# cboin1996/avddpg

Hardware: AMD Instinct MI355X
Metric: env-steps/sec + DDPG updates/sec, 4096x5-vehicle platoons (higher is better)
Workload: dtype f32-class (fp16 hi+lo operand pairs on the 16-bit matrix cores, f32 accumulate)

## Files before the change

avddpg_amd/csrc/fsplit.hip:

```cpp
#include <type_traits>

#include "fset_common.h"

namespace avd {
namespace fsplit {
using namespace fset;

struct ActorS {
    static constexpr int K = 256, KP = 256, NFT = 8, NKS = 16, LD = 264, NGT = 9, KG = 288;
    static constexpr bool critic = false;
};
struct CriticS {
    static constexpr int K = 304, KP = 320, NFT = 10, NKS = 19, LD = 312, NGT = 10, KG = 320;
    static constexpr bool critic = true;
};
constexpr int NGT_MAX = 10;

template <int I, int N, class F>
__device__ __forceinline__ void static_for(F&& f) {
    if constexpr (I < N) {
        f(std::integral_constant<int, I>{});
        static_for<I + 1, N>(f);
    }
}
// ... 273 lines not shown
            for (int k = 0; k < 4; ++k) w[k] = k < a.S ? W[k * H1 + f] : 0.f;
            b = th[(critic ? L.cbs : L.ab1) + f];
        }
        if (not_finite(w[0]) || not_finite(w[1]) || not_finite(w[2]) || not_finite(w[3]) || not_finite(b)) atomicOr(a.bad, 1);
        if (S1 * fmaxf(fmaxf(fabsf(w[0]), fabsf(w[1])), fmaxf(fmaxf(fabsf(w[2]), fabsf(w[3])), fabsf(b))) >= F16_OVERFLOW) atomicOr(a.bad, 1);
    }
    a.wf1h[net][((long)set * NGT_MAX + ft) * 64 + lane] = make_wh(w[0], w[1], w[2], w[3], b, S1, h);
    if (net == 1 && ft == 0 && lane < 48) {
        const int hl = lane / 24, hh = (lane / 12) & 1, ks = (lane / 4) % 3, m = lane & 3;
        unsigned v = 0;
#pragma unroll
        for (int e = 0; e < 2; ++e) {
            const int jj = 2 * m + e, fa = 16 * ks + 8 * (jj >> 2) + 4 * hh + (jj & 3);
            f16 hi, lo;
            split1h(S1 * th[L.cWa + fa], hi, lo);
            v |= (unsigned)__builtin_bit_cast(unsigned short, hl ? lo : hi) << (16 * e);
        }
        a.wap[(long)set * 48 + lane] = v;
    }
}

enum HeadMode { OUT_TANH = 0, OUT_TD = 1, HEAD_BOTH = 5, OUT_TANH_SAVE = 6 };
struct HeadArgs {
    unsigned long long* stamp;
    NetP net;
    int n_agents, n_sets;
    const f16x8* xf;
    const float* act;
    const float* act2;
    const float* r;
    const float* yin;
    const float* aw;
    float* out;
    f16* sm;
    float* g3;
    float* dmu;
    float* part_s;
    float* part_s2;
    float* part_m;
    float* tz;
    float gamma, high, inv_n;
    int* bad;
    int abl;
};
#ifndef HEAD_FAST
#define HEAD_FAST 5
#define HEAD_SLOW 3
#endif

template <int S, class NET, int MODE>
__global__ __launch_bounds__(NT) void head_kernel(const HeadArgs p) {
    constexpr int K = NET::K, NKS = NET::NKS, NFT = NET::NFT, LD = NET::LD;
    constexpr int NTH = NT;
    constexpr bool BOTH = (MODE == HEAD_BOTH);
    static_assert(!BOTH || NET::critic, "HEAD_BOTH is a critic mode");
    __shared__ __attribute__((aligned(16))) f16 wimg[2][H2 * LD];
    __shared__ __attribute__((aligned(16))) float b2s[H2];
    __shared__ __attribute__((aligned(16))) float c3s[H2];
    __shared__ __attribute__((aligned(16))) unsigned waps[BOTH ? 48 : 4];
    const int tid = threadIdx.x, w = tid >> 6, lane = tid & 63, r = lane & 31, h = lane >> 5, q = w >> 1, rh = w & 1;
    const int set = blockIdx.x % p.n_sets, j0 = blockIdx.x / p.n_sets, J = gridDim.x / p.n_sets, P = p.n_agents / p.n_sets;
    for (int i = tid; i < 2 * H2 * (K / 8); i += NTH) {
        const int hl = i / (H2 * (K / 8)), rem = i - hl * (H2 * (K / 8)), n = rem / (K / 8), c = rem - n * (K / 8);
        const f16* src = (hl ? p.net.Wlo : p.net.Whi) + ((long)set * H2 + n) * K + 8 * c;
        *(uint4*)(&wimg[hl][n * LD + 8 * c]) = *(const uint4*)src;
    }
    const float* vec = p.net.vec + (long)set * VEC;
// ... 63 lines not shown
            if (FSPLIT_ABL(p.abl) & 4) {
#pragma unroll
                for (int m = 0; m < 8; ++m) ph[m] = __float_as_uint(p1[2 * m]), pl[m] = __float_as_uint(p1[2 * m + 1]);
                return;
            }
#pragma unroll
            for (int m = 0; m < 8; ++m) split2h(relu(p1[2 * m]), relu(p1[2 * m + 1]), ph[m], pl[m]);
        };
        auto zdot_t = [&](f32x16& a, int t) {
            float zp = 0.f;
#pragma unroll
            for (int g = 0; g < 4; ++g) {
                const float4 c = *(const float4*)(c3s + 32 * t + 8 * g + 4 * h);
                const float cc[4] = {c.x, c.y, c.z, c.w};
#pragma unroll
                for (int j = 0; j < 4; ++j) {
                    a[4 * g + j] = relu(a[4 * g + j]);
                    zp = fmaf(a[4 * g + j], cc[j], zp);
                }
            }
            return zp;
        };
        auto zdot_nd = [&](const f32x16& a, int t) {
            float zp = 0.f;
#pragma unroll
            for (int g = 0; g < 4; ++g) {
                const float4 c = *(const float4*)(c3s + 32 * t + 8 * g + 4 * h);
                const float cc[4] = {c.x, c.y, c.z, c.w};
#pragma unroll
                for (int j = 0; j < 4; ++j) zp = fmaf(relu(a[4 * g + j]), cc[j], zp);
            }
            return zp;
        };
        auto mask_t = [&](const f32x16& a, int t, unsigned s16, f16* dst) {
            unsigned pk[4][2];
#pragma unroll
            for (int g = 0; g < 4; ++g)
#pragma unroll
                for (int e = 0; e < 2; ++e) {
                    const int i = 4 * g + 2 * e;
                    pk[g][e] = (a[i] > 0.f ? s16 : 0u) | (a[i + 1] > 0.f ? s16 << 16 : 0u);
                }
#pragma unroll
            for (int gg = 0; gg < 2; ++gg) {
                const auto s0 = __builtin_amdgcn_permlane32_swap(pk[2 * gg][0], pk[2 * gg + 1][0], false, false);
                const auto s1 = __builtin_amdgcn_permlane32_swap(pk[2 * gg][1], pk[2 * gg + 1][1], false, false);
                uint4 o;
                o.x = s0[0], o.y = s1[0], o.z = s0[1], o.w = s1[1];
                *(uint4*)(dst + 32 * t + 16 * gg) = o;
            }
        };
        auto out_z = [&](f32x16 (&ac)[4]) {
            float zp = 0.f;
#pragma unroll
            for (int t = 0; t < 4; ++t) zp += zdot_t(ac[t], t);
            zp += __shfl_xor(zp, 32);
            return d3 + zp;
        };
        split16(mfmah(wf1[0], xs, zero16));
        f16x8 wfn = wf1[64];
        f16x8 wg[2][2][2];
        auto read_group = [&](int g, f16x8 (&dst)[2][2]) {
            const int ks = g >> 1, th = g & 1;
#pragma unroll
            for (int tt = 0; tt < 2; ++tt) {
                dst[tt][0] = *(const f16x8*)(whi0 + 32 * (2 * th + tt) * LD + 16 * ks);
                dst[tt][1] = *(const f16x8*)(wlo0 + 32 * (2 * th + tt) * LD + 16 * ks);
            }
        };
        read_group(0, wg[0]);
        auto tile = [&](auto si_c, f32x16 (&ac)[4]) {
            constexpr int si = decltype(si_c)::value;
            constexpr int ft = si;
            f32x16 p1n = zero16;
            if constexpr (si + 1 < NSEQ) {
                p1n = mfmah(wfn, (NET::critic && si + 1 >= 8) ? xa : xs, zero16);
                if constexpr (si + 2 < NSEQ) wfn = wf1[64 * (si + 2)];
            }
#pragma unroll
            for (int s = 0; s < 2; ++s) {
                const int ks = 2 * ft + s;
                if (ks >= NKS) continue;
                const f16x8 bhi = fragh(ph[4 * s], ph[4 * s + 1], ph[4 * s + 2], ph[4 * s + 3]);
// ... 36 lines not shown
#pragma unroll
                for (int g = 0; g < 6; ++g) {
                    if (g + 1 < 6) read_group(2 * 16 + g + 1, wq[(g + 1) & 1]);
#pragma unroll
                    for (int tt = 0; tt < 2; ++tt) {
                        const int t = 2 * (g & 1) + tt;
                        const f16x8 whi = wq[g & 1][tt][0], wlo = wq[g & 1][tt][1];
                        c[t] = mfmah(whi, fh[g >> 1], c[t]);
                        c[t] = mfmah(wlo, fh[g >> 1], c[t]);
                        c[t] = mfmah(whi, fl[g >> 1], c[t]);
                    }
                }
            };
#pragma unroll
            for (int tl = 0; tl < 2; ++tl) {
                const f32x16 p1 = mfmah(wf1[64 * (8 + tl)], xa, zero16);
                split16(p1);
#pragma unroll
                for (int ss = 0; ss < 2 - tl; ++ss) {
                    fh[2 * tl + ss] = fragh(ph[4 * ss], ph[4 * ss + 1], ph[4 * ss + 2], ph[4 * ss + 3]);
                    fl[2 * tl + ss] = fragh(pl[4 * ss], pl[4 * ss + 1], pl[4 * ss + 2], pl[4 * ss + 3]);
                }
            }
            act_sweep(acc);
            look(acc[0][0]);
            {
                float zp = 0.f;
#pragma unroll
                for (int t = 0; t < 4; ++t) zp += zdot_nd(acc[t], t);
                zp += __shfl_xor(zp, 32);
                const float diff = d3 + zp - ty, g3a = 2.f * diff * p.inv_n * tw;
                if (h == 0) p.g3[ri] = g3a, Dacc += g3a, Lacc += diff * diff;
                gmax = fmaxf(gmax, fabsf(g3a));
#pragma unroll
                for (int t = 0; t < 4; ++t) {
                    mask_t(acc[t], t, g3a < 0.f ? 0xbc00u : 0x3c00u, p.sm + ri * H2 + 8 * h);
                }
            }
            __builtin_amdgcn_sched_barrier(0);
            f16x8 mh[3], ml[3];
#pragma unroll
            for (int tl = 0; tl < 2; ++tl) {
                const f32x16 pa = mfmah(wf1[64 * (8 + tl)], xa, zero16), pm = mfmah(wf1[64 * (8 + tl)], xb, zero16);
                unsigned dh[8], dl[8], mk[8];
#pragma unroll
                for (int m = 0; m < 4 * (2 - tl); ++m) {
                    split2h(relu(pm[2 * m]) - relu(pa[2 * m]), relu(pm[2 * m + 1]) - relu(pa[2 * m + 1]), dh[m], dl[m]);
                    mk[m] = (pm[2 * m] > 0.f ? 0xffffu : 0u) | (pm[2 * m + 1] > 0.f ? 0xffff0000u : 0u);
                }
#pragma unroll
                for (int ss = 0; ss < 2 - tl; ++ss) {
                    const int kk = 2 * tl + ss;
                    fh[kk] = fragh(dh[4 * ss], dh[4 * ss + 1], dh[4 * ss + 2], dh[4 * ss + 3]);
                    fl[kk] = fragh(dl[4 * ss], dl[4 * ss + 1], dl[4 * ss + 2], dl[4 * ss + 3]);
                    const uint4 ch = *(const uint4*)(waps + (0 * 2 + h) * 12 + 4 * kk), cl = *(const uint4*)(waps + (1 * 2 + h) * 12 + 4 * kk);
                    mh[kk] = fragh(ch.x & mk[4 * ss], ch.y & mk[4 * ss + 1], ch.z & mk[4 * ss + 2], ch.w & mk[4 * ss + 3]);
                    ml[kk] = fragh(cl.x & mk[4 * ss], cl.y & mk[4 * ss + 1], cl.z & mk[4 * ss + 2], cl.w & mk[4 * ss + 3]);
                }
            }
            act_sweep(acc);
            look(acc[0][0]);
            float zq = 0.f;
            unsigned pos[2] = {0u, 0u};
#pragma unroll
            for (int t = 0; t < 4; ++t) {
                zq += zdot_nd(acc[t], t);
#pragma unroll
                for (int i = 0; i < 16; ++i) pos[t >> 1] |= acc[t][i] > 0.f ? 1u << (16 * (t & 1) + i) : 0u;
            }
            zq += __shfl_xor(zq, 32);
            asm volatile("" : "+v"(pos[0]), "+v"(pos[1]));
#pragma unroll
            for (int kk = 0; kk < 3; ++kk) fh[kk] = mh[kk], fl[kk] = ml[kk];
#pragma unroll
            for (int t = 0; t < 4; ++t) acc[t] = zero16;
            act_sweep(acc);
            float sum = 0.f;
#pragma unroll
            for (int t = 0; t < 4; ++t)
#pragma unroll
                for (int g = 0; g < 4; ++g) {
                    const float4 c = *(const float4*)(c3s + 32 * t + 8 * g + 4 * h);
                    const float cc[4] = {c.x, c.y, c.z, c.w};
#pragma unroll
                    for (int j = 0; j < 4; ++j) sum += (pos[t >> 1] >> (16 * (t & 1) + 4 * g + j) & 1u) ? cc[j] * acc[t][4 * g + j] : 0.f;
                }
            sum += __shfl_xor(sum, 32);
            const float g3b = -p.inv_n * tw;
            if (h == 0) p.dmu[ri] = g3b * sum, Dacc2 += g3b, Lacc2 += d3 + zq;
            continue;
        }
        look(acc[0][0]);
        const float z = out_z(acc);
        if (MODE == OUT_TANH) {
            const float o = tanhf(z) * p.high;
            if (h == 0) p.out[ri] = o;
        } else if (MODE == OUT_TANH_SAVE) {
            const float t = tanhf(z);
            if (h == 0) p.out[ri] = t * p.high, p.tz[ri] = t;
#pragma unroll
            for (int tt = 0; tt < 4; ++tt) mask_t(acc[tt], tt, 0x3c00u, p.sm + ri * H2 + 8 * h);
        } else {
            if (h == 0) p.out[ri] = ty + p.gamma * z;
        }
        HSTAMP(2);
#ifdef AVD_STAMP
        if (blockIdx.x == 16 && lane == 0 && p.stamp && (w == 0 || w == 4) && ui < 28)
            p.stamp[64 + (w >> 2) * 28 + ui] = hlast - hstart;
#endif
    }
#ifdef AVD_STAMP
    if (blockIdx.x == 16 && lane == 0 && p.stamp)
        for (int i = 0; i < 4; ++i) p.stamp[w * 8 + i] = hacc[i];
#endif
    if (watch >= 0x7f800000u) atomicOr(p.bad, 1);
    if (BOTH) {
#pragma unroll
        for (int o = 1; o < 32; o <<= 1) {
            Dacc += __shfl_xor(Dacc, o), Lacc += __shfl_xor(Lacc, o);
            Dacc2 += __shfl_xor(Dacc2, o), Lacc2 += __shfl_xor(Lacc2, o);
        }
#pragma unroll
        for (int o = 1; o < 64; o <<= 1) gmax = fmaxf(gmax, __shfl_xor(gmax, o));
        if (lane == 0) {
            const long slot = (long)blockIdx.x * 8 + w;
            p.part_m[slot] = gmax;
            p.part_s[slot * 2] = Dacc, p.part_s[slot * 2 + 1] = Lacc;
            p.part_s2[slot * 2] = Dacc2, p.part_s2[slot * 2 + 1] = Lacc2;
        }
    }
}

struct SeedArgs {
    int n_agents, n_sets;
// ... 5 lines not shown
    const int tid = threadIdx.x, w = tid >> 6, lane = tid & 63;
    const int set = blockIdx.x % p.n_sets, j0 = blockIdx.x / p.n_sets, J = gridDim.x / p.n_sets, P = p.n_agents / p.n_sets;
    float gmax = 0.f, D = 0.f;
    for (int pi = j0 + w * J; pi < P; pi += 8 * J) {
        const long ri = (long)(pi * p.n_sets + set) * TILE + lane;
        const float t = p.tz[ri], g = p.dmu[ri] * p.high * (1.f - t * t);
        p.g3[ri] = g;
        gmax = fmaxf(gmax, fabsf(g));
        D += g;
    }
#pragma unroll
    for (int o = 1; o < 64; o <<= 1) gmax = fmaxf(gmax, __shfl_xor(gmax, o)), D += __shfl_xor(D, o);
    if (lane == 0) {
        p.part_m[(long)blockIdx.x * 8 + w] = gmax;
        p.part_s[((long)blockIdx.x * 8 + w) * 2] = D, p.part_s[((long)blockIdx.x * 8 + w) * 2 + 1] = 0.f;
    }
}

__device__ __forceinline__ float set_gscale(const float* part_m, int set, int n_sets, int J, float* red) {
    const int tid = threadIdx.x;
    float m = 0.f;
    for (int i = tid; i < J * 8; i += NT) m = fmaxf(m, part_m[((long)(i >> 3) * n_sets + set) * 8 + (i & 7)]);
#pragma unroll
    for (int o = 1; o < 64; o <<= 1) m = fmaxf(m, __shfl_xor(m, o));
    if ((tid & 63) == 0) red[tid >> 6] = m;
    __syncthreads();
    m = fmaxf(fmaxf(fmaxf(red[0], red[1]), fmaxf(red[2], red[3])), fmaxf(fmaxf(red[4], red[5]), fmaxf(red[6], red[7])));
    int e = 0;
    if (m > 0.f && !not_finite(m)) (void)frexpf(m, &e);
    const int k = e > 100 ? -100 : (e < -100 ? 100 : -e);
    return __uint_as_float(__builtin_amdgcn_readfirstlane(__float_as_uint(ldexpf(1.f, k))));
}

struct DwArgs {
    NetP net;
    int n_agents, n_sets;
    const float* x;
    const float* act;
    const float* g3;
    const float* part_m;
    const f16* sm;
    float* partG;
    int abl;
    unsigned long long* stamp;
};
template <int S, class NET>
__global__ __launch_bounds__(NT) void dw_kernel(const DwArgs p) {
    constexpr int KG = NET::KG, LDZ = 160;
    constexpr int XC = NET::critic ? 2 : 1;
    constexpr bool SGN = !NET::critic;
    __shared__ __attribute__((aligned(16))) unsigned short sgn16[2][TILE];
    __shared__ __attribute__((aligned(16))) f16 smimg[2][TILE * LDZ];
    __shared__ __attribute__((aligned(16))) f16x8 fq[2][TILE * 2];
    __shared__ __attribute__((aligned(16))) f16x8 fa[2][TILE * 2];
    __shared__ float gred[8];
    const int tid = threadIdx.x, w = tid >> 6, lane = tid & 63, r = lane & 31, h = lane >> 5;
    const int set = blockIdx.x % p.n_sets, j0 = blockIdx.x / p.n_sets, J = gridDim.x / p.n_sets, P = p.n_agents / p.n_sets;
    const float gsc = set_gscale(p.part_m, set, p.n_sets, J, gred);
    const f16x8* wf1 = p.net.wf1h + (long)set * NGT_MAX * 64 + lane;
    const int xt = NET::critic ? 8 + (w >> 2) : 8, xrh = NET::critic ? (w >> 1) & 1 : (w >> 2) & 1, xc0 = NET::critic ? 2 * (w & 1) : (w & 3);
    const f16x8 wf0 = wf1[64 * w], wfx = wf1[64 * xt];
    f32x16 G0[4], G1[XC];
    const f32x16 zero16 = {};
#pragma unroll
    for (int c = 0; c < 4; ++c) G0[c] = zero16;
#pragma unroll
    for (int c = 0; c < XC; ++c) G1[c] = zero16;

    const int srow = tid >> 3, sch = tid & 7, frow = tid >> 1, fh = tid & 1;
    uint4 a0 = {}, a1 = {}, b0 = {}, b1 = {};
    float sx[4] = {0.f, 0.f, 0.f, 0.f}, sg = 0.f, sa = 0.f;
    auto smsrc = [&](int pl) { return (const uint4*)(p.sm + ((long)(((FSPLIT_ABL(p.abl) & 1) ? j0 : pl) * p.n_sets + set) * TILE + srow) * H2 + 16 * sch); };
    auto fetch_x = [&](int pl) {
        if (pl >= P || tid >= 2 * TILE) return;
        const long ri = (long)(pl * p.n_sets + set) * TILE + frow;
        load_x<S>(p.x, ri, sx);
        sg = p.g3[ri];
        if (NET::critic) sa = p.act[ri];
    };
    auto stage = [&](int pl, int buf, const uint4& d0, const uint4& d1) {
        if (pl >= P) return;
        uint4* dst = (uint4*)(smimg[buf] + srow * LDZ + 16 * sch);
        dst[0] = d0, dst[1] = d1;
        if (tid < 2 * TILE) {
            const float g = fabsf(sg) * gsc;
            fq[buf][tid] = make_xg(g * sx[0], g * sx[1], g * sx[2], g * sx[3], g, fh);
            if (NET::critic) fa[buf][tid] = make_xg(g * sa, 0.f, 0.f, 0.f, g, fh);
            if (SGN && fh == 0) sgn16[buf][frow] = sg < 0.f ? 0x8000 : 0;
        }
    };
    const int g4 = lane >> 4, q = (lane & 15) >> 2, pp = lane & 3;
    typedef _Float16 f16x4 __attribute__((ext_vector_type(4)));
    auto read_tr = [&](const f16* at) {
        return __builtin_bit_cast(f16x4, __builtin_amdgcn_ds_read_tr16_b64_v4bf16((__attribute__((address_space(3))) bf16x4*)at));
    };
    auto read_b = [&](int buf, int e, int s, f16x8 (&bfr)[4]) {
#pragma unroll
        for (int c = 0; c < 4; ++c)
#pragma unroll
            for (int hf = 0; hf < 2; ++hf) {
                const int R0 = 32 * e + 16 * s + 8 * hf + 4 * (g4 >> 1);
                const f16x4 t = read_tr(smimg[buf] + (R0 + q) * LDZ + 32 * c + 16 * (g4 & 1) + 4 * pp);
#pragma unroll
                for (int j = 0; j < 4; ++j) bfr[c][4 * hf + j] = t[j];
            }
    };
    auto split16e = [&](const f32x16& p1, unsigned (&qh)[8], unsigned (&ql)[8], int buf, int e) {
        if (FSPLIT_ABL(p.abl) & 4) {
#pragma unroll
            for (int m = 0; m < 8; ++m) qh[m] = __float_as_uint(p1[2 * m]), ql[m] = __float_as_uint(p1[2 * m + 1]);
            return;
        }
#pragma unroll
        for (int m = 0; m < 8; ++m) split2h(relu(p1[2 * m]), relu(p1[2 * m + 1]), qh[m], ql[m]);
        if (SGN) {
#pragma unroll
// ... 45 lines not shown
            }
            split16e(px, ah, al, buf, xrh);
            __builtin_amdgcn_sched_group_barrier(0x008, 1, 0);
#pragma unroll
            for (int s = 0; s < 2; ++s) {
                __builtin_amdgcn_sched_group_barrier(0x100, 8, 0);
#pragma unroll
                for (int i = 0; i < 8; ++i) {
                    __builtin_amdgcn_sched_group_barrier(0x008, 1, 0);
                    __builtin_amdgcn_sched_group_barrier(0x002, SGN ? 4 : 3, 0);
                }
            }
            __builtin_amdgcn_sched_barrier(0);
        }
#pragma unroll
        for (int s = 0; s < 2; ++s) {
            const f16x8 hi = fragh(ah[4 * s], ah[4 * s + 1], ah[4 * s + 2], ah[4 * s + 3]);
            const f16x8 lo = fragh(al[4 * s], al[4 * s + 1], al[4 * s + 2], al[4 * s + 3]);
#pragma unroll
            for (int c = 0; c < XC; ++c) {
                f16x8 bx;
#pragma unroll
                for (int hf = 0; hf < 2; ++hf) {
                    const int R0 = 32 * xrh + 16 * s + 8 * hf + 4 * (g4 >> 1);
                    const f16x4 t = read_tr(smimg[buf] + (R0 + q) * LDZ + 32 * (xc0 + c) + 16 * (g4 & 1) + 4 * pp);
#pragma unroll
                    for (int j = 0; j < 4; ++j) bx[4 * hf + j] = t[j];
                }
                G1[c] = mfmah(hi, bx, G1[c]);
                G1[c] = mfmah(lo, bx, G1[c]);
            }
        }
    };
    if (j0 < P) a0 = smsrc(j0)[0], a1 = smsrc(j0)[1];
    fetch_x(j0);
    if (j0 + J < P) b0 = smsrc(j0 + J)[0], b1 = smsrc(j0 + J)[1];
    stage(j0, 0, a0, a1);
    __syncthreads();
#ifdef AVD_STAMP
    unsigned long long tacc[4] = {0, 0, 0, 0}, tlast = __builtin_amdgcn_s_memtime();
#define STAMP(i) { const unsigned long long t_ = __builtin_amdgcn_s_memtime(); tacc[i] += t_ - tlast; tlast = t_; }
#else
#define STAMP(i)
#endif
    for (int pi = j0; pi < P; pi += 2 * J) {
        fetch_x(pi + J);
        if (pi + 2 * J < P) a0 = smsrc(pi + 2 * J)[0], a1 = smsrc(pi + 2 * J)[1];
        STAMP(0);
        compute(0);
        STAMP(1);
        stage(pi + J, 1, b0, b1);
        STAMP(2);
        if (!(FSPLIT_ABL(p.abl) & 2)) __syncthreads();
        STAMP(3);
        if (pi + J < P) {
            fetch_x(pi + 2 * J);
            if (pi + 3 * J < P) b0 = smsrc(pi + 3 * J)[0], b1 = smsrc(pi + 3 * J)[1];
            STAMP(0);
            compute(1);
            STAMP(1);
            stage(pi + 2 * J, 0, a0, a1);
            STAMP(2);
            if (!(FSPLIT_ABL(p.abl) & 2)) __syncthreads();
            STAMP(3);
        }
    }
#ifdef AVD_STAMP
    if (p.stamp && blockIdx.x == 16 && lane == 0)
        for (int i = 0; i < 4; ++i) p.stamp[w * 8 + i] = tacc[i];
#endif
    const float dsc = 1.f / (gsc * S1);
    float* comb = (float*)&smimg[0][0];
    const int cidx = NET::critic ? 2 * (w >> 2) + (w & 1) : (w & 3);
    if (xrh == 1) {
#pragma unroll
        for (int c = 0; c < XC; ++c)
#pragma unroll
            for (int k = 0; k < 16; ++k) comb[((cidx * XC + c) * 16 + k) * 64 + lane] = G1[c][k];
    }
    __syncthreads();
#pragma unroll
    for (int c = 0; c < 4; ++c) {
        float* dst = p.partG + ((long)blockIdx.x * KG + 32 * w) * H2 + 32 * c + r;
#pragma unroll
        for (int k = 0; k < 16; ++k) dst[(long)acc_row(k, h) * H2] = G0[c][k] * dsc;
    }
    if (xrh == 0) {
#pragma unroll
        for (int c = 0; c < XC; ++c) {
            float* dst = p.partG + ((long)blockIdx.x * KG + 32 * xt) * H2 + 32 * (xc0 + c) + r;
#pragma unroll
            for (int k = 0; k < 16; ++k) dst[(long)acc_row(k, h) * H2] = (G1[c][k] + comb[((cidx * XC + c) * 16 + k) * 64 + lane]) * dsc;
        }
    }
}

struct DxArgs {
    NetP net;
    int n_agents, n_sets;
    const f16x8* xfh;
    const float* act;
    int L_cWa, L_cba;
    const float* g3;
    const float* part_m;
    const f16* sm;
    int unsigned_mask;
    float* partV;
    int abl;
    unsigned long long* stamp;
};
template <int S, class NET>
__global__ __launch_bounds__(NT) void dx_kernel(const DxArgs p) {
    constexpr int KP = NET::KP, LDZ = 136;
    constexpr float VSH = 1.f / 32.f;
    __shared__ __attribute__((aligned(16))) f16 smimg[2][TILE * LDZ];
    __shared__ __attribute__((aligned(16))) f16 xt[2][2][32 * 32];
    __shared__ __attribute__((aligned(16))) float g3s[2][TILE];
    __shared__ float gred[8];
    const int tid = threadIdx.x, w = __builtin_amdgcn_readfirstlane(tid >> 6), lane = tid & 63, r = lane & 31, h = lane >> 5, ft = w;
    const int set = blockIdx.x % p.n_sets, j0 = blockIdx.x / p.n_sets, J = gridDim.x / p.n_sets, P = p.n_agents / p.n_sets;
    const f32x16 zero16 = {};
    const float gsc = set_gscale(p.part_m, set, p.n_sets, J, gred);
    f16x8 wch[8], wcl[8];
    {
        const long at = ((long)set * KP + 32 * ft + r) * H2 + 8 * h;
#pragma unroll
        for (int s = 0; s < 8; ++s) wch[s] = *(const f16x8*)(p.net.Wchi + at + 16 * s), wcl[s] = *(const f16x8*)(p.net.Wclo + at + 16 * s);
    }
    const float swc = __uint_as_float(__builtin_amdgcn_readfirstlane(__float_as_uint(p.net.vec[(long)set * VEC + 2 * H2 + 2])));
    const float gv = gsc * VSH, vs = gsc * swc * VSH;
    const f16x8 wf = p.net.wf1h[((long)set * NGT_MAX + ft) * 64 + lane];
    f32x16 V = zero16;
    for (int i = tid; i < 2 * 2 * 32 * 32; i += NT) {
        const int k = (i >> 5) & 31;
        (&xt[0][0][0])[i] = (f16)(k == 8 ? 1.f : 0.f);
    }
    const int srow = tid >> 3, sch = tid & 7;
    uint4 d0 = {}, d1 = {};
    float gn = 0.f;
    auto fetch = [&](int agent) {
        if (FSPLIT_ABL(p.abl) & 1) agent = j0 * p.n_sets + set;
        const uint4* src = (const uint4*)(p.sm + ((long)agent * TILE + srow) * H2 + 16 * sch);
        d0 = src[0], d1 = src[1];
        if (tid < TILE) gn = p.g3[(long)agent * TILE + tid];
    };
    auto stage = [&](int buf) {
        uint4* dst = (uint4*)(smimg[buf] + srow * LDZ + 16 * sch);
        dst[0] = d0, dst[1] = d1;
        if (tid < TILE) g3s[buf][tid] = (p.unsigned_mask ? gn : fabsf(gn)) * gv;
    };
    f16x8 xfn0 = {}, xfn1 = {};
    auto fetch_x = [&](int agent) {
        xfn0 = p.xfh[((long)agent * TILE + r) * 2 + h];
        xfn1 = p.xfh[((long)agent * TILE + 32 + r) * 2 + h];
    };
    auto stage_x = [&](int buf) {
        if (w < 2 && h == 0) {
            f16x8 src = xfn0;
            if (w == 1) src = xfn1;
            asm volatile("" : "+v"(src));
#pragma unroll
            for (int k = 0; k < 8; ++k) xt[buf][w][k * 32 + r] = src[k];
        }
    };
    __syncthreads();
    if (j0 < P) fetch(j0 * p.n_sets + set), fetch_x(j0 * p.n_sets + set), stage(0), stage_x(0);
    __syncthreads();
#ifdef AVD_STAMP
    unsigned long long dacc[4] = {0, 0, 0, 0}, dlast = __builtin_amdgcn_s_memtime();
#define DXSTAMP(i) { const unsigned long long t_ = __builtin_amdgcn_s_memtime(); dacc[i] += t_ - dlast; dlast = t_; }
#else
#define DXSTAMP(i)
#endif
    int buf = 0;
    for (int pi = j0; pi < P; pi += J, buf ^= 1) {
        const bool more = pi + J < P;
        const f16x8 xf[2] = {xfn0, xfn1};
        if (more) fetch((pi + J) * p.n_sets + set), fetch_x((pi + J) * p.n_sets + set);
        DXSTAMP(0);
        auto read_a = [&](int e, f16x8 (&smf)[8]) {
            const f16* arow = smimg[buf] + (32 * e + r) * LDZ + 8 * h;
// ... 58 lines not shown
        for (int s = 0; s < 2; ++s) {
            V = mfmah(fragh(vh0[4 * s], vh0[4 * s + 1], vh0[4 * s + 2], vh0[4 * s + 3]), xb0[s], V);
            V = mfmah(fragh(vl0[4 * s], vl0[4 * s + 1], vl0[4 * s + 2], vl0[4 * s + 3]), xb0[s], V);
        }
        backward(1, dc1, p11, vh1, vl1);
#pragma unroll
        for (int s = 0; s < 2; ++s) {
            V = mfmah(fragh(vh1[4 * s], vh1[4 * s + 1], vh1[4 * s + 2], vh1[4 * s + 3]), xb1[s], V);
            V = mfmah(fragh(vl1[4 * s], vl1[4 * s + 1], vl1[4 * s + 2], vl1[4 * s + 3]), xb1[s], V);
        }
        DXSTAMP(1);
        if (more) stage(buf ^ 1), stage_x(buf ^ 1);
        DXSTAMP(2);
        if (!(FSPLIT_ABL(p.abl) & 2)) __syncthreads();
        DXSTAMP(3);
    }
#ifdef AVD_STAMP
    if (p.stamp && blockIdx.x == 16 && lane == 0)
        for (int i = 0; i < 4; ++i) p.stamp[w * 8 + i] = dacc[i];
#endif
    const float ivs = 1.f / vs;
    if (r < 16) {
        float* pv = p.partV + ((long)blockIdx.x * KP + 32 * ft) * 16 + r;
#pragma unroll
        for (int k = 0; k < 16; ++k) pv[(long)acc_row(k, h) * 16] = V[k] * ivs;
    }
}

template <int S>
__global__ __launch_bounds__(NT) void dxa_kernel(const DxArgs p) {
    typedef CriticS NET;
    constexpr int KP = NET::KP;
    constexpr float VSH = 1.f / 32.f;
    constexpr int LDZ = 136;
    __shared__ __attribute__((aligned(16))) f16 simg[8][32 * LDZ];
    __shared__ __attribute__((aligned(16))) float ga[8][2][2][32];
    __shared__ float comb[8][64][2];
    __shared__ float gred[8];
    const int tid = threadIdx.x, w = __builtin_amdgcn_readfirstlane(tid >> 6), lane = tid & 63, r = lane & 31, h = lane >> 5;
    const int rh = w & 1, ftl = (w >> 1) & 1, par = w >> 2;
    const int set = blockIdx.x % p.n_sets, j0 = blockIdx.x / p.n_sets, J = gridDim.x / p.n_sets, P = p.n_agents / p.n_sets;
    const f32x16 zero16 = {};
    const int ft = 8 + ftl, f = 32 * ftl + r;
    const float gsc = set_gscale(p.part_m, set, p.n_sets, J, gred);
    f16x8 wch[8], wcl[8];
    {
        const long at = ((long)set * KP + 32 * ft + r) * H2 + 8 * h;
#pragma unroll
        for (int s = 0; s < 8; ++s) wch[s] = *(const f16x8*)(p.net.Wchi + at + 16 * s), wcl[s] = *(const f16x8*)(p.net.Wclo + at + 16 * s);
    }
    const float swc = __uint_as_float(__builtin_amdgcn_readfirstlane(__float_as_uint(p.net.vec[(long)set * VEC + 2 * H2 + 2])));
    const float gv = gsc * VSH, vs = gsc * swc * VSH;
    const float* th = p.net.th + (long)set * p.net.th_stride;
    const float wa = f < HA ? th[p.L_cWa + f] : 0.f, ba = f < HA ? th[p.L_cba + f] : 0.f;
    float Sa = 0.f, Sb = 0.f;
    const int ntile = j0 < P ? (P - j0 + J - 1) / J : 0;
    uint4 A0 = {}, A1 = {}, A2 = {}, A3 = {}, A4 = {}, A5 = {}, A6 = {}, A7 = {}, B0 = {}, B1 = {}, B2 = {}, B3 = {}, B4 = {}, B5 = {}, B6 = {}, B7 = {};
    float gA = 0.f, aA = 0.f, gB = 0.f, aB = 0.f;
#define DXA_FETCH(k_, X, g_, a_)                                                                                    \
    {                                                                                                               \
        const long r0_ = (long)((j0 + (k_) * J) * p.n_sets + set) * TILE + 32 * rh;                                 \
        const uint4* src_ = (const uint4*)(p.sm + r0_ * H2) + lane;  \
        X##0 = src_[0], X##1 = src_[64], X##2 = src_[128], X##3 = src_[192], X##4 = src_[256], X##5 = src_[320], X##6 = src_[384], X##7 = src_[448]; \
        g_ = p.g3[r0_ + r], a_ = p.act[r0_ + r];                                                                    \
    }
#define DXA_PUT(buf_, X, g_, a_)                                                                                    \
    {                                                                                                               \
        if (h == 0) ga[w][buf_][0][r] = fabsf(g_) * gv, ga[w][buf_][1][r] = a_;                                     \
        f16* dst_ = simg[w] + (lane >> 4) * LDZ + 8 * (lane & 15);                                                   \
        *(uint4*)(dst_) = X##0, *(uint4*)(dst_ + 4 * LDZ) = X##1, *(uint4*)(dst_ + 8 * LDZ) = X##2, *(uint4*)(dst_ + 12 * LDZ) = X##3; \
        *(uint4*)(dst_ + 16 * LDZ) = X##4, *(uint4*)(dst_ + 20 * LDZ) = X##5, *(uint4*)(dst_ + 24 * LDZ) = X##6, *(uint4*)(dst_ + 28 * LDZ) = X##7; \
        __builtin_amdgcn_fence(__ATOMIC_RELEASE, "wavefront");                                                      \
        __builtin_amdgcn_wave_barrier();                                                                            \
    }
    auto unit = [&](int buf) {
        f32x16 dc = zero16;
        const f16* arow = simg[w] + r * LDZ + 8 * h;
#pragma unroll
        for (int s = 0; s < 8; ++s) {
            const f16x8 af = *(const f16x8*)(arow + 16 * s);
            dc = mfmah(af, wch[s], dc), dc = mfmah(af, wcl[s], dc);
        }
        float sa = 0.f, sb = 0.f;
#pragma unroll
        for (int q = 0; q < 4; ++q) {
            const float4 gq = *(const float4*)(&ga[w][buf][0][8 * q + 4 * h]), aq = *(const float4*)(&ga[w][buf][1][8 * q + 4 * h]);
            const float gg[4] = {gq.x, gq.y, gq.z, gq.w}, av[4] = {aq.x, aq.y, aq.z, aq.w};
#pragma unroll
            for (int j = 0; j < 4; ++j) {
                const float m = fmaf(av[j], wa, ba) > 0.f ? dc[4 * q + j] * gg[j] : 0.f;
                sa = fmaf(m, av[j], sa);
                sb += m;
            }
        }
        Sa += sa, Sb += sb;
        __builtin_amdgcn_fence(__ATOMIC_ACQ_REL, "wavefront");
        __builtin_amdgcn_wave_barrier();
    };
    if (par < ntile) DXA_FETCH(par, A, gA, aA);
    if (par + 2 < ntile) DXA_FETCH(par + 2, B, gB, aB);
    for (int k = par; k < ntile; k += 4) {
        DXA_PUT(0, A, gA, aA);
        if (k + 4 < ntile) DXA_FETCH(k + 4, A, gA, aA);
        unit(0);
        if (k + 2 < ntile) {
            DXA_PUT(1, B, gB, aB);
            if (k + 6 < ntile) DXA_FETCH(k + 6, B, gB, aB);
            unit(1);
        }
    }
#undef DXA_FETCH
#undef DXA_PUT
    comb[w][lane][0] = Sa, comb[w][lane][1] = Sb;
    __syncthreads();
    if (rh == 0 && par == 0 && h == 0) {
        const int ws[4] = {w, w + 1, w + 4, w + 5};
        float t[2] = {0.f, 0.f};
#pragma unroll
        for (int i = 0; i < 4; ++i)
#pragma unroll
            for (int c = 0; c < 2; ++c) t[c] += comb[ws[i]][r][c] + comb[ws[i]][32 + r][c];
        const float ivs = 1.f / vs;
        float* pv = p.partV + ((long)blockIdx.x * KP + 32 * ft + r) * 16;
#pragma unroll
        for (int c = 0; c < 9; ++c) pv[c] = c == 0 ? t[0] * ivs : (c == 8 ? t[1] * ivs : 0.f);
    }
}

struct Plan {
    int grid, J;
    size_t Whi[4], Wlo[4], Wchi[2], Wclo[2], wf1h[4], vec[4], wap, a2, y, mu, dmu, g3, sm, sma, tz, t1p, s2raw, xfs, xfs2, partHs[3], partM[2],
        partV[2], partG[2], bad, total;
};
static Plan make_plan(int n_agents, int n_sets) {
    Plan pl;
    const int P = n_agents / n_sets;
    int J = cu_count() / n_sets;
    if (const char* e = AVD_DIAG_ENV("FSPLIT_J")) J = atoi(e);
    if (J < 1) J = 1;
    if (J > P) J = P;
    pl.J = J, pl.grid = J * n_sets;
    size_t o = 0;
    auto take = [&](size_t bytes) {
        const size_t at = o;
        o += (bytes + 255) / 256 * 256;
        return at;
    };
    for (int i = 0; i < 4; ++i) {
        const int K = (i & 1) ? CriticS::K : ActorS::K, KP = (i & 1) ? CriticS::KP : ActorS::KP;
        pl.Whi[i] = take(sizeof(f16) * (size_t)n_sets * H2 * K), pl.Wlo[i] = take(sizeof(f16) * (size_t)n_sets * H2 * K);
        pl.vec[i] = take(sizeof(float) * (size_t)n_sets * VEC);
        pl.wf1h[i] = take(16 * (size_t)n_sets * NGT_MAX * 64);
        if (i < 2) pl.Wchi[i] = take(sizeof(f16) * (size_t)n_sets * KP * H2), pl.Wclo[i] = take(sizeof(f16) * (size_t)n_sets * KP * H2);
    }
    pl.wap = take(4 * (size_t)n_sets * 48);
    const size_t rows = (size_t)n_agents * TILE;
    pl.a2 = take(4 * rows), pl.y = take(4 * rows), pl.mu = take(4 * rows), pl.dmu = take(4 * rows), pl.g3 = take(4 * rows);
    pl.sm = take(sizeof(f16) * rows * H2);
    pl.sma = take(sizeof(f16) * rows * H2);
    pl.tz = take(4 * rows);
    pl.t1p = take(2 * 4 * (size_t)n_sets * CriticS::K * H2), pl.s2raw = take(2 * 4 * (size_t)n_sets * H2);
    pl.xfs = take(32 * rows), pl.xfs2 = take(32 * rows);
    for (int i = 0; i < 2; ++i) {
        const int KP = i ? CriticS::KP : ActorS::KP, KG = i ? CriticS::KG : ActorS::KG;
        pl.partM[i] = take(4 * (size_t)pl.grid * 8);
        pl.partV[i] = take(4 * (size_t)pl.grid * KP * 16);
        pl.partG[i] = take(4 * (size_t)pl.grid * KG * H2);
    }
    for (int i = 0; i < 3; ++i) pl.partHs[i] = take(4 * (size_t)pl.grid * 8 * 2);
    pl.bad = take(sizeof(int) + sizeof(unsigned) * 4 * (size_t)n_sets * 2);
    pl.total = o;
    return pl;
}
static int check_shape(const avd_mlp_layout* L, int n_agents, int n_sets, const char* who) {
    AVD_REQUIRE(L, "%s: null layout", who);
    if (L->H1 != H1 || L->H2 != H2 || L->Ha != HA || L->A != 1 || (L->S != 3 && L->S != 4) || L->B != TILE) {
        set_error("%s: serves the reference widths only (layer1 256, layer2 128, action layer 48, A = 1, S in {3, 4}, B = 64); "
                  "got H1=%d H2=%d Ha=%d A=%d S=%d B=%d (avd_learn_shared_bf16 takes other widths)",
                  who, L->H1, L->H2, L->Ha, L->A, L->S, L->B);
        return AVD_E_UNSUPPORTED;
    }
    AVD_REQUIRE(n_sets > 0 && n_sets <= 64 && n_agents > 0 && n_agents % n_sets == 0, "%s: n_agents=%d n_sets=%d", who, n_agents,
                n_sets);
    return AVD_OK;
}

enum Phase { PH_CRITIC = 1, PH_ACTOR = 2, PH_BOTH = 3 };
template <int S>
static int run(int phases, const avd_mlp_layout& L, int n_agents, int n_sets, const float* theta, const float* stats, const float* theta_t,
               const float* stats_t, const float* s, const float* a, const float* r, const float* s2, const float* aw, float gamma,
               float high, float* grads, float* losses, unsigned char* ws, const Plan& pl, hipStream_t st) {
    PrepArgs pa;
    pa.L = L, pa.S = S, pa.theta = theta, pa.stats = stats, pa.theta_t = theta_t, pa.stats_t = stats_t;
    pa.wap = (unsigned*)(ws + pl.wap), pa.bad = (int*)(ws + pl.bad), pa.smax = (unsigned*)(ws + pl.bad + sizeof(int));
    NetP net[4];
    for (int i = 0; i < 4; ++i) {
        const bool critic = i & 1, target = i >= 2;
        pa.Whi[i] = (f16*)(ws + pl.Whi[i]), pa.Wlo[i] = (f16*)(ws + pl.Wlo[i]), pa.vec[i] = (float*)(ws + pl.vec[i]);
        pa.wf1h[i] = (f16x8*)(ws + pl.wf1h[i]);
        pa.Wchi[i] = i < 2 ? (f16*)(ws + pl.Wchi[i]) : nullptr, pa.Wclo[i] = i < 2 ? (f16*)(ws + pl.Wclo[i]) : nullptr;
        NetP& n = net[i];
        n.th = (target ? theta_t : theta) + (critic ? L.actor_size : 0), n.th_stride = L.theta_size;
        n.Whi = pa.Whi[i], n.Wlo = pa.Wlo[i], n.Wchi = pa.Wchi[i], n.Wclo = pa.Wclo[i], n.wf1h = pa.wf1h[i], n.vec = pa.vec[i];
        n.wap = pa.wap;
    }
    const int P = n_agents / n_sets;
    const float inv_n = 1.0f / ((float)P * TILE);
    const long nrows = (long)n_agents * TILE;
    f16x8 *xfs = (f16x8*)(ws + pl.xfs), *xfs2 = (f16x8*)(ws + pl.xfs2);
    int* bad = (int*)(ws + pl.bad);
    float *a2 = (float*)(ws + pl.a2), *y = (float*)(ws + pl.y), *mu = (float*)(ws + pl.mu), *dmu = (float*)(ws + pl.dmu);
    float* g3 = (float*)(ws + pl.g3);
    f16 *sm = (f16*)(ws + pl.sm), *sma = (f16*)(ws + pl.sma);
    auto F = [&](size_t off) { return (float*)(ws + off); };
    const dim3 grid(pl.grid), block(NT);
    HeadArgs h;
    h.n_agents = n_agents, h.n_sets = n_sets, h.gamma = gamma, h.high = high, h.inv_n = inv_n, h.aw = aw, h.sm = sm, h.g3 = g3, h.dmu = dmu;
    h.act2 = nullptr, h.part_s2 = nullptr, h.stamp = nullptr, h.bad = bad, h.part_m = nullptr, h.tz = F(pl.tz), h.abl = 0;
    if (const char* e = AVD_DIAG_ENV("FSPLIT_ABL")) h.abl = atoi(e);
    auto head = [&](auto kern, int ni, const f16x8* x, const float* act, const float* rr, const float* yin, float* out, float* part_s) {
        h.net = net[ni], h.xf = x, h.act = act, h.r = rr, h.yin = yin, h.out = out, h.part_s = part_s;
        hipLaunchKernelGGL(kern, grid, block, 0, st, h);
    };
    DwArgs dw;
    dw.n_agents = n_agents, dw.n_sets = n_sets, dw.sm = sm, dw.g3 = g3, dw.x = s, dw.stamp = nullptr, dw.abl = 0;
    if (const char* e = AVD_DIAG_ENV("FSPLIT_ABL")) dw.abl = atoi(e);
#ifdef AVD_STAMP
    static unsigned long long* d_stamp = nullptr;
    if (!d_stamp) (void)hipMalloc(&d_stamp, 128 * 8);
    dw.stamp = d_stamp;
#endif
    DxArgs dx;
    dx.n_agents = n_agents, dx.n_sets = n_sets, dx.sm = sm, dx.g3 = g3, dx.xfh = xfs, dx.stamp = nullptr, dx.L_cWa = dx.L_cba = 0, dx.unsigned_mask = 0;
    dx.abl = dw.abl;
#ifdef AVD_STAMP
    dx.stamp = d_stamp;
#endif
    FinArgs fa;
    fa.L = L, fa.n_sets = n_sets, fa.J = pl.J, fa.S = S, fa.nrh = 1, fa.theta = theta, fa.stats = stats, fa.grads = grads, fa.losses = losses;
    fa.inv_n = inv_n, fa.partLa = F(pl.partHs[2]), fa.bad = bad;
    for (int i = 0; i < 2; ++i)
        fa.partH[i] = nullptr, fa.partHs[i] = F(pl.partHs[i]), fa.partU[i] = nullptr, fa.partV[i] = F(pl.partV[i]),
        fa.partG[i] = F(pl.partG[i]), fa.c3[i] = F(pl.vec[i]);
    fa.t1_from_g[0] = fa.t1_from_g[1] = 1, fa.t1p = F(pl.t1p), fa.s2raw = F(pl.s2raw);
    if (phases & PH_CRITIC) {
        if (hipMemsetAsync(ws + pl.bad, 0, sizeof(int) + sizeof(unsigned) * 4 * (size_t)n_sets * 2, st) != hipSuccess)
// ... 116 lines not shown
```

Before: 1.978 million.

## Store ReLU masks as packed bits instead of signed fp16 rows

The head kernel now writes the layer-2 ReLU activation masks as 128-bit bitmasks per row instead of 128 fp16 values carrying the sign of g3. The consumer kernels (dW, dV, dxa) rebuild the fp16 ±1/0 operands on the fly from the bits and the row's g3 sign via multiply tricks. The dxa kernel also drops its shared-memory staging image. This cuts mask traffic and workspace about 16x, at the cost of extra ALU unpacking in the inner loops and extra g3 loads.

```diff
diff --git a/avddpg_amd/csrc/fsplit.hip b/avddpg_amd/csrc/fsplit.hip
--- a/avddpg_amd/csrc/fsplit.hip
+++ b/avddpg_amd/csrc/fsplit.hip
@@ -329,7 +329,7 @@
     const float* yin;
     const float* aw;
     float* out;
-    f16* sm;
+    unsigned* sm;
     float* g3;
     float* dmu;
     float* part_s;
@@ -459,23 +459,20 @@
             }
             return zp;
         };
-        auto mask_t = [&](const f32x16& a, int t, unsigned s16, f16* dst) {
-            unsigned pk[4][2];
+        auto mask_t = [&](const f32x16& a) {
+            unsigned b = 0;
 #pragma unroll
             for (int g = 0; g < 4; ++g)
 #pragma unroll
-                for (int e = 0; e < 2; ++e) {
-                    const int i = 4 * g + 2 * e;
-                    pk[g][e] = (a[i] > 0.f ? s16 : 0u) | (a[i + 1] > 0.f ? s16 << 16 : 0u);
-                }
-#pragma unroll
-            for (int gg = 0; gg < 2; ++gg) {
-                const auto s0 = __builtin_amdgcn_permlane32_swap(pk[2 * gg][0], pk[2 * gg + 1][0], false, false);
-                const auto s1 = __builtin_amdgcn_permlane32_swap(pk[2 * gg][1], pk[2 * gg + 1][1], false, false);
-                uint4 o;
-                o.x = s0[0], o.y = s1[0], o.z = s0[1], o.w = s1[1];
-                *(uint4*)(dst + 32 * t + 16 * gg) = o;
-            }
+                for (int j = 0; j < 4; ++j) b |= a[4 * g + j] > 0.f ? 1u << (4 * g + (j >> 1) + 16 * (j & 1)) : 0u;
+            return b;
+        };
+        auto mask_store = [&](const unsigned (&b)[4], unsigned* dst) {
+            const auto s0 = __builtin_amdgcn_permlane32_swap(b[0], b[2], false, false);
+            const auto s1 = __builtin_amdgcn_permlane32_swap(b[1], b[3], false, false);
+            uint2 o;
+            o.x = s0[0] | (s0[1] << 2), o.y = s1[0] | (s1[1] << 2);
+            *(uint2*)(dst + 2 * h) = o;
         };
         auto out_z = [&](f32x16 (&ac)[4]) {
             float zp = 0.f;
@@ -578,10 +575,10 @@
                 const float diff = d3 + zp - ty, g3a = 2.f * diff * p.inv_n * tw;
                 if (h == 0) p.g3[ri] = g3a, Dacc += g3a, Lacc += diff * diff;
                 gmax = fmaxf(gmax, fabsf(g3a));
-#pragma unroll
-                for (int t = 0; t < 4; ++t) {
-                    mask_t(acc[t], t, g3a < 0.f ? 0xbc00u : 0x3c00u, p.sm + ri * H2 + 8 * h);
-                }
+                unsigned mb[4];
+#pragma unroll
+                for (int t = 0; t < 4; ++t) mb[t] = mask_t(acc[t]);
+                mask_store(mb, p.sm + ri * 4);
             }
             __builtin_amdgcn_sched_barrier(0);
             f16x8 mh[3], ml[3];
@@ -644,8 +641,10 @@
         } else if (MODE == OUT_TANH_SAVE) {
             const float t = tanhf(z);
             if (h == 0) p.out[ri] = t * p.high, p.tz[ri] = t;
-#pragma unroll
-            for (int tt = 0; tt < 4; ++tt) mask_t(acc[tt], tt, 0x3c00u, p.sm + ri * H2 + 8 * h);
+            unsigned mb[4];
+#pragma unroll
+            for (int tt = 0; tt < 4; ++tt) mb[tt] = mask_t(acc[tt]);
+            mask_store(mb, p.sm + ri * 4);
         } else {
             if (h == 0) p.out[ri] = ty + p.gamma * z;
         }
@@ -717,6 +716,14 @@
     return __uint_as_float(__builtin_amdgcn_readfirstlane(__float_as_uint(ldexpf(1.f, k))));
 }
 
+__device__ __forceinline__ unsigned mask_pair(unsigned d, int j, unsigned mj) { return __umul24(d & (0x10001u << j), mj); }
+__device__ __forceinline__ void mask_chunk16(unsigned w, int c, unsigned m, uint4& lo, uint4& hi) {
+    const unsigned d = w >> (8 * (c & 1));
+    lo.x = mask_pair(d, 0, m), lo.y = mask_pair(d, 1, m >> 1), lo.z = mask_pair(d, 2, m >> 2), lo.w = mask_pair(d, 3, m >> 3);
+    hi.x = mask_pair(d, 4, m >> 4), hi.y = mask_pair(d, 5, m >> 5), hi.z = mask_pair(d, 6, m >> 6), hi.w = mask_pair(d, 7, m >> 7);
+}
+__device__ __forceinline__ unsigned mask_one(float g3, bool signed_) { return signed_ && g3 < 0.f ? 0xbc00u : 0x3c00u; }
+
 struct DwArgs {
     NetP net;
     int n_agents, n_sets;
@@ -724,7 +731,7 @@
     const float* act;
     const float* g3;
     const float* part_m;
-    const f16* sm;
+    const unsigned* sm;
     float* partG;
     int abl;
     unsigned long long* stamp;
@@ -753,9 +760,13 @@
     for (int c = 0; c < XC; ++c) G1[c] = zero16;
 
     const int srow = tid >> 3, sch = tid & 7, frow = tid >> 1, fh = tid & 1;
-    uint4 a0 = {}, a1 = {}, b0 = {}, b1 = {};
-    float sx[4] = {0.f, 0.f, 0.f, 0.f}, sg = 0.f, sa = 0.f;
-    auto smsrc = [&](int pl) { return (const uint4*)(p.sm + ((long)(((FSPLIT_ABL(p.abl) & 1) ? j0 : pl) * p.n_sets + set) * TILE + srow) * H2 + 16 * sch); };
+    unsigned ma = 0, mb = 0;
+    float sx[4] = {0.f, 0.f, 0.f, 0.f}, sg = 0.f, sa = 0.f, ga = 0.f, gb = 0.f;
+    auto fetch_m = [&](int pl, unsigned& m, float& g) {
+        const long ri = (long)(((FSPLIT_ABL(p.abl) & 1) ? j0 : pl) * p.n_sets + set) * TILE + srow;
+        m = p.sm[ri * 4 + (sch >> 1)];
+        if (NET::critic) g = p.g3[ri];
+    };
     auto fetch_x = [&](int pl) {
         if (pl >= P || tid >= 2 * TILE) return;
         const long ri = (long)(pl * p.n_sets + set) * TILE + frow;
@@ -763,10 +774,10 @@
         sg = p.g3[ri];
         if (NET::critic) sa = p.act[ri];
     };
-    auto stage = [&](int pl, int buf, const uint4& d0, const uint4& d1) {
+    auto stage = [&](int pl, int buf, unsigned m, float g) {
         if (pl >= P) return;
         uint4* dst = (uint4*)(smimg[buf] + srow * LDZ + 16 * sch);
-        dst[0] = d0, dst[1] = d1;
+        mask_chunk16(m, sch, mask_one(g, NET::critic), dst[0], dst[1]);
         if (tid < 2 * TILE) {
             const float g = fabsf(sg) * gsc;
             fq[buf][tid] = make_xg(g * sx[0], g * sx[1], g * sx[2], g * sx[3], g, fh);
@@ -878,10 +889,10 @@
             }
         }
     };
-    if (j0 < P) a0 = smsrc(j0)[0], a1 = smsrc(j0)[1];
+    if (j0 < P) fetch_m(j0, ma, ga);
     fetch_x(j0);
-    if (j0 + J < P) b0 = smsrc(j0 + J)[0], b1 = smsrc(j0 + J)[1];
-    stage(j0, 0, a0, a1);
+    if (j0 + J < P) fetch_m(j0 + J, mb, gb);
+    stage(j0, 0, ma, ga);
     __syncthreads();
 #ifdef AVD_STAMP
     unsigned long long tacc[4] = {0, 0, 0, 0}, tlast = __builtin_amdgcn_s_memtime();
@@ -891,21 +902,21 @@
 #endif
     for (int pi = j0; pi < P; pi += 2 * J) {
         fetch_x(pi + J);
-        if (pi + 2 * J < P) a0 = smsrc(pi + 2 * J)[0], a1 = smsrc(pi + 2 * J)[1];
+        if (pi + 2 * J < P) fetch_m(pi + 2 * J, ma, ga);
         STAMP(0);
         compute(0);
         STAMP(1);
-        stage(pi + J, 1, b0, b1);
+        stage(pi + J, 1, mb, gb);
         STAMP(2);
         if (!(FSPLIT_ABL(p.abl) & 2)) __syncthreads();
         STAMP(3);
         if (pi + J < P) {
             fetch_x(pi + 2 * J);
-            if (pi + 3 * J < P) b0 = smsrc(pi + 3 * J)[0], b1 = smsrc(pi + 3 * J)[1];
+            if (pi + 3 * J < P) fetch_m(pi + 3 * J, mb, gb);
             STAMP(0);
             compute(1);
             STAMP(1);
-            stage(pi + 2 * J, 0, a0, a1);
+            stage(pi + 2 * J, 0, ma, ga);
             STAMP(2);
             if (!(FSPLIT_ABL(p.abl) & 2)) __syncthreads();
             STAMP(3);
@@ -949,7 +960,7 @@
     int L_cWa, L_cba;
     const float* g3;
     const float* part_m;
-    const f16* sm;
+    const unsigned* sm;
     int unsigned_mask;
     float* partV;
     int abl;
@@ -982,17 +993,17 @@
         (&xt[0][0][0])[i] = (f16)(k == 8 ? 1.f : 0.f);
     }
     const int srow = tid >> 3, sch = tid & 7;
-    uint4 d0 = {}, d1 = {};
-    float gn = 0.f;
+    unsigned dm = 0;
+    float gn = 0.f, gs = 0.f;
     auto fetch = [&](int agent) {
         if (FSPLIT_ABL(p.abl) & 1) agent = j0 * p.n_sets + set;
-        const uint4* src = (const uint4*)(p.sm + ((long)agent * TILE + srow) * H2 + 16 * sch);
-        d0 = src[0], d1 = src[1];
+        dm = p.sm[((long)agent * TILE + srow) * 4 + (sch >> 1)];
+        if (NET::critic) gs = p.g3[(long)agent * TILE + srow];
         if (tid < TILE) gn = p.g3[(long)agent * TILE + tid];
     };
     auto stage = [&](int buf) {
         uint4* dst = (uint4*)(smimg[buf] + srow * LDZ + 16 * sch);
-        dst[0] = d0, dst[1] = d1;
+        mask_chunk16(dm, sch, mask_one(gs, NET::critic), dst[0], dst[1]);
         if (tid < TILE) g3s[buf][tid] = (p.unsigned_mask ? gn : fabsf(gn)) * gv;
     };
     f16x8 xfn0 = {}, xfn1 = {};
@@ -1117,8 +1128,6 @@
     typedef CriticS NET;
     constexpr int KP = NET::KP;
     constexpr float VSH = 1.f / 32.f;
-    constexpr int LDZ = 136;
-    __shared__ __attribute__((aligned(16))) f16 simg[8][32 * LDZ];
     __shared__ __attribute__((aligned(16))) float ga[8][2][2][32];
     __shared__ float comb[8][64][2];
     __shared__ float gred[8];
@@ -1140,30 +1149,28 @@
     const float wa = f < HA ? th[p.L_cWa + f] : 0.f, ba = f < HA ? th[p.L_cba + f] : 0.f;
     float Sa = 0.f, Sb = 0.f;
     const int ntile = j0 < P ? (P - j0 + J - 1) / J : 0;
-    uint4 A0 = {}, A1 = {}, A2 = {}, A3 = {}, A4 = {}, A5 = {}, A6 = {}, A7 = {}, B0 = {}, B1 = {}, B2 = {}, B3 = {}, B4 = {}, B5 = {}, B6 = {}, B7 = {};
+    uint4 mA = {}, mB = {};
     float gA = 0.f, aA = 0.f, gB = 0.f, aB = 0.f;
-#define DXA_FETCH(k_, X, g_, a_)                                                                                    \
+#define DXA_FETCH(k_, m_, g_, a_)                                                                                   \
     {                                                                                                               \
         const long r0_ = (long)((j0 + (k_) * J) * p.n_sets + set) * TILE + 32 * rh;                                 \
-        const uint4* src_ = (const uint4*)(p.sm + r0_ * H2) + lane;  \
-        X##0 = src_[0], X##1 = src_[64], X##2 = src_[128], X##3 = src_[192], X##4 = src_[256], X##5 = src_[320], X##6 = src_[384], X##7 = src_[448]; \
+        m_ = *(const uint4*)(p.sm + (r0_ + r) * 4);                                                                 \
         g_ = p.g3[r0_ + r], a_ = p.act[r0_ + r];                                                                    \
     }
-#define DXA_PUT(buf_, X, g_, a_)                                                                                    \
+#define DXA_PUT(buf_, g_, a_)                                                                                       \
     {                                                                                                               \
         if (h == 0) ga[w][buf_][0][r] = fabsf(g_) * gv, ga[w][buf_][1][r] = a_;                                     \
-        f16* dst_ = simg[w] + (lane >> 4) * LDZ + 8 * (lane & 15);                                                   \
-        *(uint4*)(dst_) = X##0, *(uint4*)(dst_ + 4 * LDZ) = X##1, *(uint4*)(dst_ + 8 * LDZ) = X##2, *(uint4*)(dst_ + 12 * LDZ) = X##3; \
-        *(uint4*)(dst_ + 16 * LDZ) = X##4, *(uint4*)(dst_ + 20 * LDZ) = X##5, *(uint4*)(dst_ + 24 * LDZ) = X##6, *(uint4*)(dst_ + 28 * LDZ) = X##7; \
         __builtin_amdgcn_fence(__ATOMIC_RELEASE, "wavefront");                                                      \
         __builtin_amdgcn_wave_barrier();                                                                            \
     }
-    auto unit = [&](int buf) {
+    auto unit = [&](int buf, const uint4 mw, float g) {
         f32x16 dc = zero16;
-        const f16* arow = simg[w] + r * LDZ + 8 * h;
+        const unsigned m = mask_one(g, true);
+        const unsigned mwt[4] = {mw.x >> (4 * h), mw.y >> (4 * h), mw.z >> (4 * h), mw.w >> (4 * h)};
 #pragma unroll
         for (int s = 0; s < 8; ++s) {
-            const f16x8 af = *(const f16x8*)(arow + 16 * s);
+            const unsigned d = mwt[s >> 1] >> (8 * (s & 1));
+            const f16x8 af = fragh(mask_pair(d, 0, m), mask_pair(d, 1, m >> 1), mask_pair(d, 2, m >> 2), mask_pair(d, 3, m >> 3));
             dc = mfmah(af, wch[s], dc), dc = mfmah(af, wcl[s], dc);
         }
         float sa = 0.f, sb = 0.f;
@@ -1182,16 +1189,22 @@
         __builtin_amdgcn_fence(__ATOMIC_ACQ_REL, "wavefront");
         __builtin_amdgcn_wave_barrier();
     };
-    if (par < ntile) DXA_FETCH(par, A, gA, aA);
-    if (par + 2 < ntile) DXA_FETCH(par + 2, B, gB, aB);
+    if (par < ntile) DXA_FETCH(par, mA, gA, aA);
+    if (par + 2 < ntile) DXA_FETCH(par + 2, mB, gB, aB);
     for (int k = par; k < ntile; k += 4) {
-        DXA_PUT(0, A, gA, aA);
-        if (k + 4 < ntile) DXA_FETCH(k + 4, A, gA, aA);
-        unit(0);
+        DXA_PUT(0, gA, aA);
+        {
+            const uint4 mc = mA;
+            const float gc = gA;
+            if (k + 4 < ntile) DXA_FETCH(k + 4, mA, gA, aA);
+            unit(0, mc, gc);
+        }
         if (k + 2 < ntile) {
-            DXA_PUT(1, B, gB, aB);
-            if (k + 6 < ntile) DXA_FETCH(k + 6, B, gB, aB);
-            unit(1);
+            DXA_PUT(1, gB, aB);
+            const uint4 mc = mB;
+            const float gc = gB;
+            if (k + 6 < ntile) DXA_FETCH(k + 6, mB, gB, aB);
+            unit(1, mc, gc);
         }
     }
 #undef DXA_FETCH
@@ -1241,8 +1254,8 @@
     pl.wap = take(4 * (size_t)n_sets * 48);
     const size_t rows = (size_t)n_agents * TILE;
     pl.a2 = take(4 * rows), pl.y = take(4 * rows), pl.mu = take(4 * rows), pl.dmu = take(4 * rows), pl.g3 = take(4 * rows);
-    pl.sm = take(sizeof(f16) * rows * H2);
-    pl.sma = take(sizeof(f16) * rows * H2);
+    pl.sm = take(16 * rows);
+    pl.sma = take(16 * rows);
     pl.tz = take(4 * rows);
     pl.t1p = take(2 * 4 * (size_t)n_sets * CriticS::K * H2), pl.s2raw = take(2 * 4 * (size_t)n_sets * H2);
     pl.xfs = take(32 * rows), pl.xfs2 = take(32 * rows);
@@ -1296,7 +1309,7 @@
     int* bad = (int*)(ws + pl.bad);
     float *a2 = (float*)(ws + pl.a2), *y = (float*)(ws + pl.y), *mu = (float*)(ws + pl.mu), *dmu = (float*)(ws + pl.dmu);
     float* g3 = (float*)(ws + pl.g3);
-    f16 *sm = (f16*)(ws + pl.sm), *sma = (f16*)(ws + pl.sma);
+    unsigned *sm = (unsigned*)(ws + pl.sm), *sma = (unsigned*)(ws + pl.sma);
     auto F = [&](size_t off) { return (float*)(ws + off); };
     const dim3 grid(pl.grid), block(NT);
     HeadArgs h;
```

Result: faster. 2.046 million (median of 6 runs) (+3.5%).
